# XJTU-Power-AI/charginghub-env

Measured on AMD Instinct MI355X. Metric: env-steps/sec at 65 536 parallel envs, higher is better.
Workload: dtype f64; 1 GPU; 65536 envs x hub [20 fast, 25 slow] (BASELINE.json configs[3]), fcev_permeate 0.01, random policy resident in HBM, reset every 96 steps, Philox streams; envs_per_gpu=65536, obs_dim=13, act_dim=47, work_order=XCD-aware (tiles, tail and level workgroups in contiguous eighths per XCD), graph=on, collective=none

## Files before the change

### charginghub-env_amd/csrc/chub_kernels.hip

```cpp
#include <hip/hip_runtime.h>
#include <hip/hip_ext.h>
#include <stdint.h>

#include "chub_device.h"
#include "chub_plan.h"

namespace chub {

typedef uint32_t u32x4 __attribute__((ext_vector_type(4)));
typedef uint32_t u32x2 __attribute__((ext_vector_type(2)));

__device__ __forceinline__ bool in_group(const StepArgs &sa, int64_t env) { return !sa.env_mask || sa.env_mask[env] != 0; }
__device__ __forceinline__ uint32_t env_clk(const StepArgs &sa, int64_t n_envs, int64_t env) {
    return sa.env_clk[(int64_t) (sa.tick & 1u) * n_envs + env];
}
__device__ __forceinline__ int64_t range_len(const StepArgs &sa) { return (int64_t) sa.env_hi - sa.env_lo + 1; }
__device__ __forceinline__ bool range_unit(const StepArgs &sa, int64_t i, int segments, int &seg, int64_t &env) {
    const int64_t R = range_len(sa);
    if (i >= (int64_t) segments * R) return false;
    seg = (i >= R ? 1 : 0) + (i >= 2 * R ? 1 : 0);
    env = sa.env_lo + (i - (int64_t) seg * R);
    return true;
}

// ... 2617 lines not shown

struct NoMid {
    __device__ __forceinline__ void operator()() {}
    __device__ __forceinline__ void at1() {}
    __device__ __forceinline__ void at2() {}
    __device__ __forceinline__ void at3() {}
};
__device__ __forceinline__ uint32_t hv_count_rate(float rate, uint32_t n) {
    const int c = (int) roundf(rate * (float) n);
    return (uint32_t) (c < 0 ? 0 : (c > 255 ? 255 : c));
}
__device__ __forceinline__ uint32_t hv_count_env(const EnvParamArrays &ep, uint32_t e, int t, uint32_t lev) {
    return hv_count_rate(ep.hv_rate[e], (uint32_t) ep.hv_idx[(uint32_t) t * (uint32_t) kLevels + lev]);
}

template <bool RESET, int MODE, bool MULTI, bool FUSED = false, typename Mid = NoMid, int EB = kEnvBlock, bool TAPE = false, bool EP = false, int PAIR = 0>
__device__ __forceinline__ void env_tail(const DevCtx *__restrict__ ctx, const StepArgs &sa, const int env, const bool live,
                                         const double *s_pv, const double *s_wd, const double *s_pv_now, const double *s_wd_now,
                                         const double *s_hy, const uint8_t *s_hv, float *s_out, const int env_block, const TailArgs &ta,
                                         const u32x4 *s_rec, const int local_env, const int env0_fused, const int rows_fused,
                                         const TailIn &pre, const bool use_pre, Mid &mid, TailNext *nx = nullptr, const TailArgs *ta2 = nullptr) {
    static_assert(PAIR == 0 || (!RESET && MODE == MODE_PHILOX && !MULTI && !FUSED && !TAPE && !EP), "pairs: the lock-step PHILOX step of the stand-alone tail");
    const HubParams &hp = ctx->hp;
    const EnvArrays &ev = ctx->ev;
    const CompatRng &cr = ctx->cr;
    const Tables &tb = ctx->tb;
    const int64_t N = hp.n_envs;
    constexpr bool multi = MULTI;
    const uint32_t my_clk = (multi && env < (int) N) ? env_clk(sa, N, env) : 0u;
    if (multi && env < (int) N)
        sa.env_clk[(int64_t) ((sa.tick + 1u) & 1u) * N + env] = (uint16_t) (!live ? my_clk : (RESET ? 0u : clk_next(my_clk)));
    const int t_now = multi ? clk_t(my_clk) : sa.t;
    const int t_next = RESET ? 0 : (t_now + 1) % 96;
    const bool draw_price = multi ? ((my_clk >> 8) & 3u) == 0u : sa.draw_price != 0;
    const double price_last = multi ? tb.price[RESET ? 95 : t_now] : sa.price_last;
    const double price_prev = multi ? tb.price[(t_now + 95) % 96] : sa.price_prev;
#define TAB_PV(d) (multi ? tb.pvT[t_next * 100 + (d)] : s_pv[d])
// ... 9 lines not shown
    CHUB_STAMP(0);
#if CHUB_TRACE
    {
        uint32_t n_ = n32;
        asm volatile("" : "+s"(n_));
        CHUB_STAMP(1);
    }
#endif
    double st_pv = 0.0, st_wd = 0.0, st_hy = 0.0, st_pv_now = 0.0, st_wd_now = 0.0;
    uint32_t st_hv = 0;
    const double sin_t = multi ? tb.sin96[t_next] : ta.sin_t;
    const int32_t tel_word = hp.telemetry;
    const bool tel_on = (tel_word & 1) != 0;
    const bool ep_on = (tel_word & 2) != 0;
    if (!FUSED) {
        const int i = threadIdx.x;
        if (PAIR == 2) {
            st_pv = nx->st_pv;
            st_wd = nx->st_wd;
        } else if (!multi) {
            if (i < 100) st_pv = ta.pv_row[i];
            if (i < 150) st_wd = ta.wd_row[i];
            if (!RESET) {
                if (i < 100) st_pv_now = ta.pv_row_now[i];
                if (i < 150) st_wd_now = ta.wd_row_now[i];
            }
            if (PAIR == 1) {
                nx->st_pv = nx->st_wd = 0.0;
                if (i < 100) nx->st_pv = ta2->pv_row[i];
                if (i < 150) nx->st_wd = ta2->wd_row[i];
            }
        }
        if (!RESET && PAIR != 2) {
            if (!EP && i < 102) st_hy = ta.hy_table[i];
            if (MODE == MODE_COMPAT && !EP && !multi && !sa.hv_tape && i < kLevels / 4) st_hv = ((CHUB_G(const uint32_t)) tb.cnt_hv)[sa.t * (kLevels / 4) + i];
        }
    }
    constexpr bool tick_late = MODE == MODE_PHILOX && !RESET && !TAPE;
    const bool tick_now = MODE == MODE_PHILOX && (!tick_late || sa.fresh != 0);
    PhiloxCtx px{ta.key[0], ta.key[1], tick_now ? sa.tick + sload_u32(ta.tick_base, 0) : sa.tick, ta.gid0 + (uint32_t) env};
    double cap = 0.0, in_price_noise = 0.0;
    double ou_pv = 0.0, ou_wd = 0.0, ou_price = 0.0, z_pv = 0.0, z_wd = 0.0, z_pr = 0.0;
    float a_el_f = 0.0f, a_fc_f = 0.0f, P0f = 0.0f, P1f = 0.0f, mn0 = 0.0f, mx0 = 0.0f, mn1 = 0.0f, mx1 = 0.0f;
    int pv_day = 0, wd_day = 0, q_len = 0, hv_line = 0, F0i = 0, F1i = 0, ln0 = 0, ln1 = 0, hv_lev = 0, hv_arrive = 0;
    u32x4 drw_raw = {0u, 0u, 0u, 0u};
    uint32_t drw_n = 0u, hvw0 = 0u, hvw1 = 0u;
    const bool have_pre = (FUSED || PAIR == 2) && use_pre;
    double p_v_h_max = 0.0, p_cells = 0.0, p_rc_cells = 0.0, p_cap_mass = 0.0, p_rc_cap_mass = 0.0, p_init_soc = 0.0, p_hydro_loss = 0.0;
    double p_fc_max_power = 0.0, p_renew_fluct1 = 0.0, p_price_fluct1 = 0.0;
// ... 4 lines not shown
            p_renew_fluct1 = pr[PRM_RENEW_FLUCT1 * n32 + e32];
            p_price_fluct1 = pr[PRM_PRICE_FLUCT1 * n32 + e32];
            if (RESET) {
                p_init_soc = pr[PRM_INIT_SOC * n32 + e32];
            } else {
                p_v_h_max = pr[PRM_V_H_MAX * n32 + e32];
                p_cells = pr[PRM_CELLS * n32 + e32];
                p_rc_cells = pr[PRM_RC_CELLS * n32 + e32];
                p_rc_cap_mass = pr[PRM_RC_CAP_MASS * n32 + e32];
                p_hydro_loss = pr[PRM_HYDRO_LOSS * n32 + e32];
                p_fc_max_power = pr[PRM_FC_MAX_POWER * n32 + e32];
            }
        }
        if (have_pre) {
            ou_pv = pre.ou_pv; ou_wd = pre.ou_wd; ou_price = pre.ou_price; in_price_noise = pre.price_noise;
        } else {
            ou_pv = ta.ou[e32];
            ou_wd = ta.ou[n32 + e32];
            ou_price = ta.ou[2u * n32 + e32];
            in_price_noise = ta.price_noise[e32];
        }
        if (PAIR == 2) {
            const u32x4 v0 = nx->r0, v1 = nx->r1;
            mn0 = __uint_as_float(v0.x); P0f = __uint_as_float(v0.y); mx0 = __uint_as_float(v0.z); ln0 = pkd_line(v0.w); F0i = pkd_flow(v0.w);
            mn1 = __uint_as_float(v1.x); P1f = __uint_as_float(v1.y); mx1 = __uint_as_float(v1.z); ln1 = pkd_line(v1.w); F1i = pkd_flow(v1.w);
        } else if (!FUSED) {
            const StationRec r0 = rec_load(ta.rec, e32), r1 = rec_load(ta.rec, n32 + e32);
            mn0 = r0.mn; P0f = r0.chg; mx0 = r0.mx; ln0 = pkd_line(r0.pkd); F0i = pkd_flow(r0.pkd);
            mn1 = r1.mn; P1f = r1.chg; mx1 = r1.mx; ln1 = pkd_line(r1.pkd); F1i = pkd_flow(r1.pkd);
        }
        if (!RESET && have_pre) {
            a_el_f = pre.a_el; a_fc_f = pre.a_fc; cap = pre.cap;
            pv_day = pre.pv_day; wd_day = pre.wd_day; q_len = pre.q_len; hv_line = pre.hv_line;
        } else if (!RESET) {
            if (ta.tail_act) {
                typedef float f32x2_ __attribute__((ext_vector_type(2)));
                const f32x2_ tv = ((CHUB_G(const f32x2_)) ta.tail_act)[e32];
                a_el_f = tv.x;
                a_fc_f = tv.y;
            } else {
                const uint32_t ai = e32 * ta.act_dim + ta.s_tot;
                a_el_f = ta.actions[ai];
                a_fc_f = ta.actions[ai + 1u];
            }
            cap = ta.cap[e32];
            pv_day = ta.pv_day[e32];
            wd_day = ta.wd_day[e32];
            q_len = ta.q_len[e32];
            hv_line = ta.hv_line[e32];
        }
        if (MODE == MODE_COMPAT && !RESET && sa.hv_tape) {
            hvw0 = sa.hv_tape[e32 * (uint32_t) sa.hv_w];
            if (sa.hv_w > 1) hvw1 = sa.hv_tape[e32 * (uint32_t) sa.hv_w + 1u];
        }
        if (TAPE) {
            z_pv = sa.exo_z[e32 * 3u + 0u];
            z_wd = sa.exo_z[e32 * 3u + 1u];
            z_pr = sa.exo_z[e32 * 3u + 2u];
            if (!RESET) hv_arrive = (int) sa.hv_tape[e32 * (uint32_t) sa.hv_w];
        } else if (MODE == MODE_PHILOX && !RESET && !sa.fresh) {
            if (have_pre) {
                drw_raw = pre.drw;
                drw_n = pre.drw_n;
            } else {
                drw_raw = ((CHUB_G(const u32x4)) ta.drw)[e32];
                drw_n = ta.drw_cnt[e32];
            }
        } else if (MODE == MODE_PHILOX) {
            const U4 ow = px.block(SITE_OU, 0, 0);
            z_pv = (double) normal_from_word(tb.normal_icdf, tb.normal_tail, ow.v[0]);
            z_wd = (double) normal_from_word(tb.normal_icdf, tb.normal_tail, ow.v[1]);
            z_pr = (double) normal_from_word(tb.normal_icdf, tb.normal_tail, ow.v[2]);
            if (!RESET) {
                hv_lev = (int) (px.block(SITE_HV, 0, 0).v[0] % 1000u);
                hv_arrive = EP ? (int) hv_count_env(ctx->ep, e32, t_now, (uint32_t) hv_lev)
                               : (int) tb.cnt_hv[(uint32_t) t_now * (uint32_t) kLevels + (uint32_t) hv_lev];
            }
        } else {
            z_pv = sa.exo_z[e32 * 3u + 0u];
            z_wd = sa.exo_z[e32 * 3u + 1u];
            z_pr = sa.exo_z[e32 * 3u + 2u];
        }
        if (PAIR == 1) {
            typedef float f32x2_ __attribute__((ext_vector_type(2)));
            nx->r0 = ((CHUB_G(const u32x4)) ta2->rec)[e32];
            nx->r1 = ((CHUB_G(const u32x4)) ta2->rec)[n32 + e32];
            const f32x2_ tv = ((CHUB_G(const f32x2_)) ta2->tail_act)[e32];
            nx->in.a_el = tv.x;
            nx->in.a_fc = tv.y;
            nx->in.drw = ((CHUB_G(const u32x4)) ta2->drw)[e32];
            nx->in.drw_n = ta2->drw_cnt[e32];
        }
    }


    if (tick_late && !tick_now) {
        const uint32_t *tbp = ta.tick_base;
        asm volatile("" : "+s"(tbp) : : "memory");
        px.tick += sload_u32(tbp, 0);
    }
    if (!FUSED) {
        static_assert(EB >= 150, "one table element per lane");
        CHUB_STAMP(2);
        const int i = threadIdx.x;
        if (i < 100) ((double *) s_pv)[i] = st_pv;
        if (i < 150) ((double *) s_wd)[i] = st_wd;
        if (!RESET && PAIR != 2) {
            if (i < 100) ((double *) s_pv_now)[i] = st_pv_now;
            if (i < 150) ((double *) s_wd_now)[i] = st_wd_now;
            if (!EP && i < 102) ((double *) s_hy)[i] = st_hy;
            if (MODE == MODE_COMPAT && !EP && i < kLevels / 4) ((uint32_t *) s_hv)[i] = st_hv;
        }
        __syncthreads();
    }
    CHUB_STAMP(3);
    if (!TAPE && MODE == MODE_PHILOX && !RESET && !sa.fresh) {
        z_pv = (double) __uint_as_float(drw_raw.x);
        z_wd = (double) __uint_as_float(drw_raw.y);
        z_pr = (double) __uint_as_float(drw_raw.z);
        hv_arrive = (int) drw_n;
    }
    const int row_w = sa.obs_stride;
    auto flush_rows = [&]() {
        if (FUSED) {
            __builtin_amdgcn_fence(__ATOMIC_RELEASE, "wavefront");
            __builtin_amdgcn_wave_barrier();
// ... 6 lines not shown
                for (int i = (int) (threadIdx.x & 63u); i < quads; i += 64) ((f32x4 *) dst)[i] = ((const f32x4 *) s_out)[i];
                for (int i = (quads << 2) + (int) (threadIdx.x & 63u); i < total; i += 64) dst[i] = s_out[i];
            } else {
                for (int i = (int) (threadIdx.x & 63u); i < total; i += 64) dst[i] = s_out[i];
            }
            __builtin_amdgcn_fence(__ATOMIC_RELEASE, "wavefront");
            __builtin_amdgcn_wave_barrier();
            return;
        }
        __syncthreads();
        const int env0 = env_block * EB;
        const int rows = (int) N - env0 < EB ? (int) N - env0 : EB;
        float *dst = sa.obs + (size_t) env0 * (size_t) row_w;
        const int total = rows * row_w;
        if (MULTI && sa.env_mask && !__syncthreads_and((live || env >= (int) N) ? 1 : 0)) {
            for (int i = threadIdx.x; i < total; i += EB)
                if (in_group(sa, env0 + i / row_w)) dst[i] = s_out[i];
        } else if ((((uintptr_t) dst) & 15u) == 0) {
            typedef float f32x4 __attribute__((ext_vector_type(4)));
            const int quads = total >> 2;
            for (int i = threadIdx.x; i < quads; i += EB) ((f32x4 *) dst)[i] = ((const f32x4 *) s_out)[i];
            for (int i = (quads << 2) + threadIdx.x; i < total; i += EB) dst[i] = s_out[i];
        } else {
            for (int i = threadIdx.x; i < total; i += EB) dst[i] = s_out[i];
        }
    };
    const double *hy_env = (MODE == MODE_COMPAT || EP) ? (const double *) ev.hy_env + (size_t) e32 * 102u : nullptr;
    (void) hy_env;
    double hy_req_pre = 0.0;
    if ((MODE == MODE_COMPAT || EP) && !RESET && live) {
        int rq = (int) ceil((((double) a_el_f + 1) / 2) * 100);
        rq = rq < 0 ? 0 : (rq > 101 ? 101 : rq);
        hy_req_pre = hy_env[rq];
    }
    const double cap_mass = HP_E(cap_mass, p_cap_mass);
    double store_soc = 0.0, reward = 0.0, in_re_pv = 0.0, in_re_wd = 0.0, in_price_next = 0.0, total_mass_need = 0.0;
    double re_pv = 0.0, re_wd = 0.0, price_next = 0.0;
    int arrive = 0;
    uint32_t fold_n = 0;
    do {
    if (!live) break;

    const bool hv_walked = MODE == MODE_COMPAT && sa.hv_tape != nullptr;
    CompatStream rs;
    if (MODE == MODE_COMPAT && !RESET && !hv_walked) rs.load(cr, sa.rng_cur, env);

    if (RESET) {
        if (MODE == MODE_COMPAT || TAPE) {
            pv_day = sa.exo_days[e32 * 2u + 0u];
            wd_day = sa.exo_days[e32 * 2u + 1u];
        } else {
            const U4 o = px.block(SITE_DAY, 0, 0);
            pv_day = (int) (o.v[0] % 100u);
            wd_day = (int) (o.v[1] % 150u);
        }
        ev.pv_day[e32] = (int16_t) pv_day;
// ... 131 lines not shown
        if (draw_price) {
            price_next = ou_sample(ou_price, .1, 0.005, z_pr) * HP_E(price_fluct1, p_price_fluct1);
            ev.ou[2u * n32 + e32] = ou_price;
            ev.price_noise[e32] = price_next;
            if (PAIR == 1) nx->in.price_noise = price_next;
            price_next += price_last;
        } else {
            price_next = price_last + in_price_noise;
            if (PAIR == 1) nx->in.price_noise = in_price_noise;
        }
    }
    if (MODE == MODE_COMPAT && !RESET && !hv_walked) rs.store(cr, sa.rng_cur, env);
    } while (0);

    CHUB_STAMP(4);
    mid();
    if (FUSED && live) {
        const u32x4 v0 = s_rec[2 * local_env], v1 = s_rec[2 * local_env + 1];
        mn0 = __uint_as_float(v0.x); P0f = __uint_as_float(v0.y); mx0 = __uint_as_float(v0.z); ln0 = pkd_line(v0.w); F0i = pkd_flow(v0.w);
        mn1 = __uint_as_float(v1.x); P1f = __uint_as_float(v1.y); mx1 = __uint_as_float(v1.z); ln1 = pkd_line(v1.w); F1i = pkd_flow(v1.w);
    }

    do {
    if (!live) break;
    if (!RESET) {
        const double a_el = ((double) a_el_f + 1) / 2;
        const double a_fc = ((double) a_fc_f + 1) / 2;
        const double P0 = (double) P0f, P1 = (double) P1f;
        const double F0 = (double) F0i, F1 = (double) F1i;
        double re_new_power = in_re_wd + in_re_pv;
        const double charging_power = 0.0 + P0 + P1;
// ... 85 lines not shown
        const double hy_loss = -6 / 1000.0 * hy_to_use;
        const double real_price_dollar = in_price_next / 4;
        const double income_evs_fast = 0.42 / 4 * P0 - real_price_dollar * e0;
        const double income_evs_slow = 0.21 / 4 * P1 - real_price_dollar * e1;
        const double income_evs = income_evs_fast + income_evs_slow;
        const double income_evs_serve = 0.8 * (0.0 + F0 + F1);
        const double income_hys = 6 / 1000.0 * hy_use;
        const double not_meet_loss = -10 / 1000.0 * not_meet;
        const double hy_cost = -real_price_dollar * hydrogen_power;
        reward = DIV_K(income_hys + income_evs + income_evs_serve + hy_cost + 1 * hy_loss + not_meet_loss, 50);
        if (tel_on) {
            CHUB_TEL(0, act_el); CHUB_TEL(1, flow); CHUB_TEL(2, all_power_second); CHUB_TEL(4, cap);
            CHUB_TEL(5, total_mass_need); CHUB_TEL(6, hy_use); CHUB_TEL(7, not_meet); CHUB_TEL(8, fc_power);
            CHUB_TEL(9, hy_to_use); CHUB_TEL(10, used_renew); CHUB_TEL(13, hydrogen_power);
            CHUB_TEL(14, income_hys + income_evs + income_evs_serve + hy_cost); CHUB_TEL(15, reward);
            CHUB_TEL(19, (double) arrive); CHUB_TEL(20, (double) hv_line); CHUB_TEL(21, (double) q_len + (double) fold_n);
            CHUB_TEL(24, e0); CHUB_TEL(25, e1); CHUB_TEL(26, ev_power_sum);
            CHUB_TEL(27, in_price_next);
        }
        if (ep_on) {
            CHUB_G(double) lv = ctx->es.live;
            const size_t nn = n32, ee = e32;
            const double init_soc = EP ? ctx->ep.prm[PRM_INIT_SOC * n32 + e32] : hp.init_soc;
            double col[kEpCount];
            col[EPC_RETURN] = lv[EPC_RETURN * nn + ee] + reward;
            col[EPC_INCOME] = lv[EPC_INCOME * nn + ee] + (income_hys + income_evs + income_evs_serve + hy_cost);
            col[EPC_DRAW_ELE] = lv[EPC_DRAW_ELE * nn + ee] + ((e0 + e1) + hydrogen_power);
            col[EPC_LENGTH] = lv[EPC_LENGTH * nn + ee] + 1.0;
            col[EPC_DEVIATION] = fabs(store_soc - init_soc);
            col[EPC_TEST_PENALTY] = fabs(col[EPC_DEVIATION] * cap_mass / 1000 / 0.2);
            col[EPC_END_SOC] = store_soc;
// ... 8 lines not shown
            }
        }
        }
    }

    ev.cap[e32] = cap;
    if (PAIR == 1) {
        nx->in.ou_pv = ou_pv;
        nx->in.ou_wd = ou_wd;
        nx->in.ou_price = ou_price;
        nx->in.cap = cap;
        nx->in.pv_day = pv_day;
        nx->in.wd_day = wd_day;
    }

    float *obs = s_out + (FUSED ? (int) (threadIdx.x & 63u) : (int) threadIdx.x) * row_w;
    double *o64 = tel_on ? (double *) ev.obs64 + (size_t) e32 * hp.obs_dim : nullptr;
    int n = 0;
#define CHUB_OBS(v)                    \
    do {                               \
        const double v_ = (v);         \
        obs[n] = (float) v_;           \
        if (o64) o64[n] = v_;          \
        n++;                           \
    } while (0)
    CHUB_OBS(sin_t);
    CHUB_OBS(div_c(price_next - hp.price_mean, hp.price_std, hp.rc_price_std));
    if (hp.S[0] > 0) {
        const double half_range = (double) hp.transformer_limit[0] / 2, rc_hr = hp.rc_half_range[0];
        CHUB_OBS(div_c((double) mn0 - half_range, half_range, rc_hr));
        CHUB_OBS(div_c((double) P0f - half_range, half_range, rc_hr));
// ... 16 lines not shown
        if (sa.done_f32) {
            obs[n] = (float) reward;
            obs[n + 1] = dn ? 1.0f : 0.0f;
        } else {
            sa.reward[(size_t) e32 * sa.reward_stride] = (float) reward;
            if (sa.done) sa.done[e32] = (uint8_t) (dn ? 1 : 0);
            if (sa.done_f32) sa.done_f32[(size_t) e32 * sa.reward_stride] = dn ? 1.0f : 0.0f;
        }
    } else if (MULTI && sa.done_f32) {
        obs[n] = sa.reward[(size_t) e32 * sa.reward_stride];
        obs[n + 1] = sa.done_f32[(size_t) e32 * sa.reward_stride];
    }
    if (tel_on) {
        ev.reward64[e32] = reward;
        CHUB_TEL(3, store_soc); CHUB_TEL(16, re_pv); CHUB_TEL(17, re_wd); CHUB_TEL(18, price_next);
        CHUB_TEL(22, (double) pv_day); CHUB_TEL(23, (double) wd_day);
        CHUB_TEL(28, (double) mn0); CHUB_TEL(29, (double) P0f); CHUB_TEL(30, (double) mx0); CHUB_TEL(31, (double) ln0); CHUB_TEL(32, (double) F0i);
        CHUB_TEL(33, (double) mn1); CHUB_TEL(34, (double) P1f); CHUB_TEL(35, (double) mx1); CHUB_TEL(36, (double) ln1); CHUB_TEL(37, (double) F1i);
    }
    } while (0);
    CHUB_STAMP(5);
    mid.at3();
    if (MULTI) {
        if (RESET && sa.final_obs && live) {
            const float *row = sa.obs + (size_t) e32 * (size_t) row_w;
            float *fin = sa.final_obs + (size_t) e32 * (size_t) hp.obs_dim;
            for (int j = 0; j < hp.obs_dim; j++) fin[j] = row[j];
        }
        if (sa.tick_note && live) sa.tick_note[e32] = CHUB_TICK(hp, sa.tick);
        if (!RESET && sa.done_mask) {
            const bool dn = live && (t_now + 1) >= 96;
            if (env < (int) N) sa.done_mask[e32] = (uint8_t) (dn ? 1 : 0);
            const unsigned long long fired = __ballot(dn);
            if ((threadIdx.x & 63u) == 0u && fired != 0ull) atomicAdd(sa.done_count, (uint32_t) __popcll(fired));
        }
    }
    flush_rows();
#if CHUB_TRACE
    CHUB_STAMP(6);
    asm volatile("s_waitcnt vmcnt(0)" ::: "memory");
    CHUB_STAMP(7);
    CHUB_STAMP_REAL(9);
    if (!FUSED && sa.stamps_env && threadIdx.x == 0) for (int i = 0; i < 10; i++) sa.stamps_env[(size_t) env_block * 16 + i] = stamp_[i];
#endif
#undef TAB_PV
#undef TAB_WD
#undef TAB_PV_NOW
#undef TAB_WD_NOW
#undef TAB_HY
#undef TAB_HV
#undef HP_E
}

template <bool RESET, bool MULTI, bool EP = false>
__device__ __forceinline__ void level_block(const DevCtx *__restrict__ ctx, const StepArgs &sa, const int64_t u, const int line_known = -1) {
    const HubParams &hp = ctx->hp;
    const int64_t N = hp.n_envs;
    if (u >= 3 * N) return;
// ... 78 lines not shown
    const HubParams &hp = ctx->hp;
    const Tables &tb = ctx->tb;
    PhiloxCtx px{hp.key[0], hp.key[1], tick, (uint32_t) (hp.env_id0 + e)};
    const U4 ow = px.block(SITE_OU, 0, 0);
    const uint32_t hv_lev = px.block(SITE_HV, 0, 0).v[0] % 1000u;
    u32x4 d;
    d.x = __float_as_uint(normal_from_word(tb.normal_icdf, tb.normal_tail, ow.v[0]));
    d.y = __float_as_uint(normal_from_word(tb.normal_icdf, tb.normal_tail, ow.v[1]));
    d.z = __float_as_uint(normal_from_word(tb.normal_icdf, tb.normal_tail, ow.v[2]));
    const uint32_t cnt = (uint32_t) tb.cnt_hv[(uint32_t) t * (uint32_t) kLevels + hv_lev];
    d.w = cnt != 0u ? __float_as_uint(soc_from_word(tb.soc_d_icdf, px.block(SITE_HVSOC, 0, 0).v[0])) : 0u;
    ((CHUB_G(u32x4)) drw)[e] = d;
    cnt_out[e] = (uint8_t) cnt;
}

__device__ __forceinline__ bool level_lane(const uint32_t jb, const uint32_t n32, const int nb_env, const uint32_t xcd, int64_t &u) {
    const uint32_t per = n32 >> 3;
    if (xcd && (n32 & 2047u) == 0u && ((uint32_t) nb_env & 7u) == 0u) {
        const uint32_t x = jb & 7u, i = jb >> 3, wpx = per / kEnvBlock;
        const uint32_t seg = i / wpx;
        u = (int64_t) seg * n32 + (int64_t) (x * per + (i - seg * wpx) * kEnvBlock + threadIdx.x);
        return seg < 3u;
    }
    u = (int64_t) jb * kEnvBlock + threadIdx.x;
    return u < 3 * (int64_t) n32;
}

__global__ __launch_bounds__(kEnvBlock) void k_pair_draws(const DevCtx *__restrict__ ctx, StepArgs sa, PairArgs pr, uint32_t xcd) {
    const HubParams &hp = ctx->hp;
    const uint32_t n32 = (uint32_t) hp.n_envs;
    int64_t u;
    if (!level_lane(blockIdx.x, n32, 8, xcd, u)) return;
    const uint32_t tick1 = CHUB_TICK(hp, sa.tick + 1u);
    if (u < 2 * (int64_t) n32) {
        const int kk = u >= (int64_t) n32 ? 1 : 0;
        const int want = dk_want(ctx->st.pk[sa.tick & 1u][u]);
        pr.pkraw[u] = draw_raw_levels(hp, ctx->tb, tick1, sa.t + 1, kk, u - (int64_t) kk * n32, want, hp.type[kk] == 0);
    } else {
        const uint32_t e = (uint32_t) (u - 2 * (int64_t) n32);
        draw_env_pre(ctx, tick1 - 1u, sa.t, e, pr.drw_out[0], pr.cnt_out[0]);
        draw_env_pre(ctx, tick1, sa.t + 1, e, pr.drw_out[1], pr.cnt_out[1]);
    }
}

template <bool MORE>
__global__ __launch_bounds__(kEnvBlock) void k_env_pair(const DevCtx *__restrict__ ctx, StepArgs sa, StepArgs sb, TailArgs ta, TailArgs tb2, PairArgs pr,
                                                        int nb_env) {
    __shared__ double s_pv[100], s_wd[150], s_pv_now[100], s_wd_now[150], s_hy[102], s_pv2[100], s_wd2[150];
    __shared__ __attribute__((aligned(16))) float s_out[2][kEnvBlock * 16];
    if ((int) blockIdx.x >= nb_env) {
        const HubParams &hp = ctx->hp;
        const uint32_t n32 = (uint32_t) hp.n_envs;
        int64_t u;
        if (!level_lane(blockIdx.x - (uint32_t) nb_env, n32, nb_env, ta.xcd, u)) return;
        if (!MORE) {
            level_block<false, false>(ctx, sb, u);
            if (u < 2 * (int64_t) n32) {
                const int kk = u >= (int64_t) n32 ? 1 : 0;
                ctx->st.pk[sb.tick & 1u][u] = dk_make(pr.pkraw[u], pkd_line(pr.rec_a[4u * (uint32_t) u + 3u]), hp.type[kk] == 0);
            } else {
                const uint32_t e = (uint32_t) (u - 2 * (int64_t) n32);
                ((CHUB_G(u32x4)) ctx->ev.drw[sb.tick & 1u])[e] = ((CHUB_G(const u32x4)) pr.drw_in[1])[e];
                ctx->ev.drw_cnt[sb.tick & 1u][e] = pr.cnt_in[1][e];
            }
            return;
        }
        const uint32_t tick2 = CHUB_TICK(hp, sb.tick + 1u);
        if (u < 2 * (int64_t) n32) {
            const int kk = u >= (int64_t) n32 ? 1 : 0;
            const bool fast = hp.type[kk] == 0;
            const int64_t env_ = u - (int64_t) kk * n32;
            const int line_now = pkd_line(ctx->st.rec[4u * (uint32_t) u + 3u]);
            const uint32_t dk = draw_decoded_levels(hp, ctx->tb, tick2, sb.t + 1, kk, env_, line_now, fast);
            ctx->st.pk[(sb.tick + 1u) & 1u][u] = dk;
            pr.pkraw[u] = draw_raw_levels(hp, ctx->tb, tick2 + 1u, sb.t + 2, kk, env_, dk_want(dk), fast);
        } else {
            const uint32_t e = (uint32_t) (u - 2 * (int64_t) n32);
            draw_env_pre(ctx, tick2, sb.t + 1, e, pr.drw_out[0], pr.cnt_out[0]);
            draw_env_pre(ctx, tick2 + 1u, sb.t + 2, e, pr.drw_out[1], pr.cnt_out[1]);
        }
        return;
    }
    const int blk = (int) xcd_order(blockIdx.x, (uint32_t) nb_env, ta.xcd);
    const int env = blk * kEnvBlock + (int) threadIdx.x;
    const bool live = env < (int) ta.n_envs;
    TailIn none;
    TailNext nx;
    NoMid nomid;
    env_tail<false, MODE_PHILOX, false, false, NoMid, kEnvBlock, false, false, 1>(ctx, sa, env, live, s_pv, s_wd, s_pv_now, s_wd_now, s_hy, nullptr, s_out[0], blk, ta,
                                                                                  nullptr, 0, 0, 0, none, false, nomid, &nx, &tb2);
    env_tail<false, MODE_PHILOX, false, false, NoMid, kEnvBlock, false, false, 2>(ctx, sb, env, live, s_pv2, s_wd2, s_pv, s_wd, s_hy, nullptr, s_out[1], blk, tb2,
                                                                                  nullptr, 0, 0, 0, nx.in, true, nomid, &nx, nullptr);
}

__global__ __launch_bounds__(256) void k_env_walk(const DevCtx *__restrict__ ctx, StepArgs sa, TailArgs ta, StepArgs sw, int nb_env) {
    __shared__ __attribute__((aligned(16))) uint32_t lds[32 * 256 + 4 * kWalkStageWords];
    if ((int) blockIdx.x >= nb_env) {
        __builtin_amdgcn_s_setprio(3);
        compat_walk_block<false>(ctx, sw, blockIdx.x - (uint32_t) nb_env, lds, lds + 32 * 256);
        return;
    }
    double *s_pv = (double *) lds, *s_wd = s_pv + 100, *s_pv_now = s_wd + 150, *s_wd_now = s_pv_now + 100, *s_hy = s_wd_now + 150;
    uint8_t *s_hv = (uint8_t *) (s_hy + 102 + 2);
    float *s_out = (float *) (s_hv + 1008);
    static_assert((602 + 2) * 8 + 1008 + kEnvBlock * 16 * 4 <= 32 * 256 * 4 && kLevels <= 1008, "the tail's LDS inside the walk's");
    const int env = (int) blockIdx.x * kEnvBlock + (int) threadIdx.x;
    TailIn none;
// ... 1580 lines not shown
template void launch_env<false>(EnvForm, const HubParams &, const DevCtx *, const StepArgs &, hipStream_t, hipEvent_t, hipEvent_t, const PackedPtrs &);

void launch_env_walk(const HubParams &hp, const DevCtx *ctx, const StepArgs &sa, const StepArgs &sw, hipStream_t stream, hipEvent_t ev0, hipEvent_t ev1,
                     const PackedPtrs &pp) {
    const TailArgs ta = make_tail_args(*pp.ev, *pp.st, hp, sa, pp, false);
    const int nb_env = (int) ((hp.n_envs + kEnvBlock - 1) / kEnvBlock);
    const unsigned nb = (unsigned) nb_env + (unsigned) ((hp.n_envs + 255) / 256);
    CHUB_LAUNCH(k_env_walk, dim3(nb), dim3(kEnvBlock), stream, ev0, ev1, ctx, sa, ta, sw, nb_env);
}

void launch_pair(const HubParams &hp, const DevCtx *ctx, const StepArgs &sa_in, const StepArgs &sb_in, hipStream_t stream, const PackedPtrs &pp,
                 const PairBufs &pb, int sel, bool chain_start, bool more) {
    StepArgs sa = sa_in, sb = sb_in;
    const int64_t N = hp.n_envs;
    const int nb_env = (int) ((N + kEnvBlock - 1) / kEnvBlock);
    const unsigned nb_lev = (unsigned) ((3 * N + kEnvBlock - 1) / kEnvBlock);
    PairArgs pr;
    pr.rec_a = (CHUB_G(const uint32_t)) pb.rec_a;
    pr.pkraw = (CHUB_G(uint64_t)) pb.pkraw;
    for (int q = 0; q < 2; q++) {
        pr.drw_in[q] = (CHUB_G(const uint32_t)) pb.drw[sel][q];
        pr.cnt_in[q] = (CHUB_G(const uint8_t)) pb.cnt[sel][q];
        pr.drw_out[q] = (CHUB_G(uint32_t)) pb.drw[sel ^ 1][q];
        pr.cnt_out[q] = (CHUB_G(uint8_t)) pb.cnt[sel ^ 1][q];
    }
    const uint32_t xcd = hp.xcd ? 1u : 0u;
    if (chain_start) {
        launch_levels(sa.fresh ? LEVELS_DRAW : LEVELS_NONE, ctx, sa, stream);
        PairArgs p0 = pr;
        for (int q = 0; q < 2; q++) {
            p0.drw_out[q] = (CHUB_G(uint32_t)) pb.drw[sel][q];
            p0.cnt_out[q] = (CHUB_G(uint8_t)) pb.cnt[sel][q];
        }
        hipLaunchKernelGGL(k_pair_draws, dim3(nb_lev), dim3(kEnvBlock), 0, stream, ctx, sa, p0, xcd);
    }
    sa.fresh = 0;
    sb.fresh = 0;
    const uint32_t nb = (uint32_t) ((N + hp.epb - 1) / hp.epb);
    PackedArgs pa = make_packed_args(hp, sa, pp);
    pa.rec = (CHUB_G(uint32_t)) pb.rec_a;
    pa.tail_act = (CHUB_G(float)) pb.tail_act_a;
    hipLaunchKernelGGL((k_slot_packed<kPackedBlock, kSlotsPerLane, false, false, false, false>), dim3(nb), dim3(kPackedBlock), 0, stream, ctx, sa, pa);
    PackedArgs pa2 = make_packed_args(hp, sb, pp);
    pa2.pk = (CHUB_G(const uint32_t)) (const void *) pb.pkraw;
    pa2.rec_prev = (CHUB_G(const uint32_t)) pb.rec_a;
    hipLaunchKernelGGL((k_slot_packed<kPackedBlock, kSlotsPerLane, false, false, false, false, false, true>), dim3(nb), dim3(kPackedBlock), 0, stream, ctx,
                       sb, pa2);
    TailArgs ta = make_tail_args(*pp.ev, *pp.st, hp, sa, pp, false), tb2 = make_tail_args(*pp.ev, *pp.st, hp, sb, pp, false);
    ta.rec = (CHUB_G(uint32_t)) pb.rec_a;
    ta.tail_act = (CHUB_G(const float)) pb.tail_act_a;
    ta.drw = pr.drw_in[0];
    ta.drw_cnt = pr.cnt_in[0];
    tb2.drw = pr.drw_in[1];
    tb2.drw_cnt = pr.cnt_in[1];
    if (more) hipLaunchKernelGGL(k_env_pair<true>, dim3((unsigned) nb_env + nb_lev), dim3(kEnvBlock), 0, stream, ctx, sa, sb, ta, tb2, pr, nb_env);
    else hipLaunchKernelGGL(k_env_pair<false>, dim3((unsigned) nb_env + nb_lev), dim3(kEnvBlock), 0, stream, ctx, sa, sb, ta, tb2, pr, nb_env);
}

__global__ void k_tick_advance(uint32_t *tick_base, uint32_t by) { *tick_base += by; }


__global__ void k_expand_bits(int64_t n_envs, int S, int W, const uint64_t *__restrict__ bits, const float *__restrict__ tail,
                              float *__restrict__ actions) {
    const uint32_t A = (uint32_t) S + 2u;
    const uint32_t total = (uint32_t) n_envs * A;
    for (uint32_t i = blockIdx.x * blockDim.x + threadIdx.x; i < total; i += gridDim.x * blockDim.x) {
        const uint32_t env = i / A;
        const uint32_t j = i - env * A;
        float v;
        if (j < (uint32_t) S) v = ((bits[(size_t) env * (size_t) W + (j >> 6)] >> (j & 63u)) & 1ull) ? 1.0f : -1.0f;
        else v = tail[env * 2u + (j - (uint32_t) S)];
// ... 251 lines not shown
```

### charginghub-env_amd/csrc/chub_runtime.cpp

```cpp
#include <hip/hip_runtime.h>
#include <math.h>
#include <stdint.h>
#include <stdio.h>
#include <string.h>
#include <stdlib.h>

#include <algorithm>
#include <map>
#include <string>
#include <vector>

#include "../../include/chub.h"
#include "chub_device.h"
#include "chub_plan.h"
#include "chub_policy.h"
#include "chub_critic.h"
#include "chub_adam.h"

namespace chub {
template <bool RESET>
void launch_slot(const CallPlan &cp, const HubParams &hp, const LaunchPlan &lp, const DevCtx *ctx, const StepArgs &sa, hipStream_t stream,
                 const PackedPtrs &pp, hipEvent_t ev0, hipEvent_t ev1);
void launch_check_ttab(const DevCtx *ctx, uint32_t *d_mismatch, hipStream_t stream);
void launch_build_cls_soc(const DevCtx *ctx, float *d_out, hipStream_t stream);
// ... 1652 lines not shown
        const StepCall c2 = step_call(nullptr, batches[(i + 1) % n_batches], nullptr, packed_out(e, packed2[(i + 1) & 1]), 0);
        StepArgs sa, sb;
        if (const int rc = fill_args(e, c1, 2, all, e->tick + 1u, s, sa)) return rc;
        {
            const int t0 = e->t, pc0 = e->price_count;
            const bool pd0 = e->predrawn;
            e->t = t0 + 1;
            e->price_count = pc0 + 1;
            e->predrawn = true;
            const int rc = fill_args(e, c2, 2, all, e->tick + 2u, s, sb);
            e->t = t0;
            e->price_count = pc0;
            e->predrawn = pd0;
            if (rc) return rc;
        }
        launch_pair(e->hp, e->d_ctx, sa, sb, s, packed_ptrs(e), e->pair, sel, p == 0, p + 1 < n_pairs);
        if (hipGetLastError() != hipSuccess) {
            e->predrawn = false;
            return fail(CHUB_ERR_HIP, "a pair of steps could not be launched");
        }
        e->tick += 2u;
        advance_clocks(e, c1, 2, 2);
        sel ^= 1;
    }
    return note_served(e, nullptr, 2, s);
}

int chub_run_steps(chub_env *e, chub_comm *comm, const float *const *d_action_batches, int n_batches, float *const *d_packed2,
                   float *const *d_gathered2, float *d_reset_obs, int64_t first_step, int64_t n_steps, void *stream) {
    if (!e || !d_action_batches || n_batches <= 0 || !d_packed2 || !d_packed2[0] || !d_packed2[1] || !d_reset_obs || first_step < 0 ||
// ... 3623 lines not shown
```

Measured before the change: 2.747 billion env-steps/s.

## Split pair tail across two role halves of a doubled workgroup

The paired-step kernel now launches workgroups twice as wide. One half (role 1) runs the first part of each env's tail: loading tables, computing renewables, price and mass need, and writing them to shared memory. The other half (role 2) loads station records, actions and hydrogen tables, then takes over the rest of the step after a barrier. This splits each env's serial work across two wavefront groups and lets more memory loads be in flight at once. It adds barriers and shared-memory hand-over traffic. The level and draw kernels also use the larger block size.

```diff
diff --git a/charginghub-env_amd/csrc/chub_kernels.hip b/charginghub-env_amd/csrc/chub_kernels.hip
--- a/charginghub-env_amd/csrc/chub_kernels.hip
+++ b/charginghub-env_amd/csrc/chub_kernels.hip
@@ -2655,13 +2655,22 @@
     return hv_count_rate(ep.hv_rate[e], (uint32_t) ep.hv_idx[(uint32_t) t * (uint32_t) kLevels + lev]);
 }
 
-template <bool RESET, int MODE, bool MULTI, bool FUSED = false, typename Mid = NoMid, int EB = kEnvBlock, bool TAPE = false, bool EP = false, int PAIR = 0>
+struct PairSplit {
+    double *s_pv2, *s_wd2;
+    double *hand;
+};
+template <bool RESET, int MODE, bool MULTI, bool FUSED = false, typename Mid = NoMid, int EB = kEnvBlock, bool TAPE = false, bool EP = false, int PAIR = 0,
+          int ROLE = 0>
 __device__ __forceinline__ void env_tail(const DevCtx *__restrict__ ctx, const StepArgs &sa, const int env, const bool live,
                                          const double *s_pv, const double *s_wd, const double *s_pv_now, const double *s_wd_now,
                                          const double *s_hy, const uint8_t *s_hv, float *s_out, const int env_block, const TailArgs &ta,
                                          const u32x4 *s_rec, const int local_env, const int env0_fused, const int rows_fused,
-                                         const TailIn &pre, const bool use_pre, Mid &mid, TailNext *nx = nullptr, const TailArgs *ta2 = nullptr) {
+                                         const TailIn &pre, const bool use_pre, Mid &mid, TailNext *nx = nullptr, const TailArgs *ta2 = nullptr,
+                                         const PairSplit *ps = nullptr) {
     static_assert(PAIR == 0 || (!RESET && MODE == MODE_PHILOX && !MULTI && !FUSED && !TAPE && !EP), "pairs: the lock-step PHILOX step of the stand-alone tail");
+    static_assert(ROLE == 0 || PAIR != 0, "roles: the halves of a pair's steps");
+    const int tid = ROLE ? (int) (threadIdx.x & (uint32_t) (EB - 1)) : (int) threadIdx.x;
+    (void) tid;
     const HubParams &hp = ctx->hp;
     const EnvArrays &ev = ctx->ev;
     const CompatRng &cr = ctx->cr;
@@ -2701,11 +2710,11 @@
     const bool tel_on = (tel_word & 1) != 0;
     const bool ep_on = (tel_word & 2) != 0;
     if (!FUSED) {
-        const int i = threadIdx.x;
+        const int i = tid;
         if (PAIR == 2) {
             st_pv = nx->st_pv;
             st_wd = nx->st_wd;
-        } else if (!multi) {
+        } else if (!multi && ROLE != 2) {
             if (i < 100) st_pv = ta.pv_row[i];
             if (i < 150) st_wd = ta.wd_row[i];
             if (!RESET) {
@@ -2719,7 +2728,7 @@
             }
         }
         if (!RESET && PAIR != 2) {
-            if (!EP && i < 102) st_hy = ta.hy_table[i];
+            if (ROLE != 1 && !EP && i < 102) st_hy = ta.hy_table[i];
             if (MODE == MODE_COMPAT && !EP && !multi && !sa.hv_tape && i < kLevels / 4) st_hv = ((CHUB_G(const uint32_t)) tb.cnt_hv)[sa.t * (kLevels / 4) + i];
         }
     }
@@ -2754,7 +2763,7 @@
         }
         if (have_pre) {
             ou_pv = pre.ou_pv; ou_wd = pre.ou_wd; ou_price = pre.ou_price; in_price_noise = pre.price_noise;
-        } else {
+        } else if (ROLE != 2) {
             ou_pv = ta.ou[e32];
             ou_wd = ta.ou[n32 + e32];
             ou_price = ta.ou[2u * n32 + e32];
@@ -2764,7 +2773,7 @@
             const u32x4 v0 = nx->r0, v1 = nx->r1;
             mn0 = __uint_as_float(v0.x); P0f = __uint_as_float(v0.y); mx0 = __uint_as_float(v0.z); ln0 = pkd_line(v0.w); F0i = pkd_flow(v0.w);
             mn1 = __uint_as_float(v1.x); P1f = __uint_as_float(v1.y); mx1 = __uint_as_float(v1.z); ln1 = pkd_line(v1.w); F1i = pkd_flow(v1.w);
-        } else if (!FUSED) {
+        } else if (!FUSED && ROLE != 1) {
             const StationRec r0 = rec_load(ta.rec, e32), r1 = rec_load(ta.rec, n32 + e32);
             mn0 = r0.mn; P0f = r0.chg; mx0 = r0.mx; ln0 = pkd_line(r0.pkd); F0i = pkd_flow(r0.pkd);
             mn1 = r1.mn; P1f = r1.chg; mx1 = r1.mx; ln1 = pkd_line(r1.pkd); F1i = pkd_flow(r1.pkd);
@@ -2773,7 +2782,8 @@
             a_el_f = pre.a_el; a_fc_f = pre.a_fc; cap = pre.cap;
             pv_day = pre.pv_day; wd_day = pre.wd_day; q_len = pre.q_len; hv_line = pre.hv_line;
         } else if (!RESET) {
-            if (ta.tail_act) {
+            if (ROLE == 1) {
+            } else if (ta.tail_act) {
                 typedef float f32x2_ __attribute__((ext_vector_type(2)));
                 const f32x2_ tv = ((CHUB_G(const f32x2_)) ta.tail_act)[e32];
                 a_el_f = tv.x;
@@ -2783,11 +2793,13 @@
                 a_el_f = ta.actions[ai];
                 a_fc_f = ta.actions[ai + 1u];
             }
-            cap = ta.cap[e32];
-            pv_day = ta.pv_day[e32];
-            wd_day = ta.wd_day[e32];
-            q_len = ta.q_len[e32];
-            hv_line = ta.hv_line[e32];
+            if (ROLE != 1) cap = ta.cap[e32];
+            if (ROLE != 2) {
+                pv_day = ta.pv_day[e32];
+                wd_day = ta.wd_day[e32];
+                q_len = ta.q_len[e32];
+                hv_line = ta.hv_line[e32];
+            }
         }
         if (MODE == MODE_COMPAT && !RESET && sa.hv_tape) {
             hvw0 = sa.hv_tape[e32 * (uint32_t) sa.hv_w];
@@ -2802,7 +2814,7 @@
             if (have_pre) {
                 drw_raw = pre.drw;
                 drw_n = pre.drw_n;
-            } else {
+            } else if (ROLE != 2) {
                 drw_raw = ((CHUB_G(const u32x4)) ta.drw)[e32];
                 drw_n = ta.drw_cnt[e32];
             }
@@ -2823,33 +2835,45 @@
         }
         if (PAIR == 1) {
             typedef float f32x2_ __attribute__((ext_vector_type(2)));
-            nx->r0 = ((CHUB_G(const u32x4)) ta2->rec)[e32];
-            nx->r1 = ((CHUB_G(const u32x4)) ta2->rec)[n32 + e32];
-            const f32x2_ tv = ((CHUB_G(const f32x2_)) ta2->tail_act)[e32];
-            nx->in.a_el = tv.x;
-            nx->in.a_fc = tv.y;
-            nx->in.drw = ((CHUB_G(const u32x4)) ta2->drw)[e32];
-            nx->in.drw_n = ta2->drw_cnt[e32];
-        }
-    }
-
-
-    if (tick_late && !tick_now) {
+            if (ROLE != 1) {
+                nx->r0 = ((CHUB_G(const u32x4)) ta2->rec)[e32];
+                nx->r1 = ((CHUB_G(const u32x4)) ta2->rec)[n32 + e32];
+                const f32x2_ tv = ((CHUB_G(const f32x2_)) ta2->tail_act)[e32];
+                nx->in.a_el = tv.x;
+                nx->in.a_fc = tv.y;
+            }
+            if (ROLE != 2) {
+                nx->in.drw = ((CHUB_G(const u32x4)) ta2->drw)[e32];
+                nx->in.drw_n = ta2->drw_cnt[e32];
+            }
+        }
+    }
+
+
+    if (tick_late && !tick_now && ROLE != 2) {
         const uint32_t *tbp = ta.tick_base;
         asm volatile("" : "+s"(tbp) : : "memory");
         px.tick += sload_u32(tbp, 0);
     }
-    if (!FUSED) {
+    if (!FUSED && !(ROLE != 0 && PAIR == 2)) {
         static_assert(EB >= 150, "one table element per lane");
         CHUB_STAMP(2);
-        const int i = threadIdx.x;
-        if (i < 100) ((double *) s_pv)[i] = st_pv;
-        if (i < 150) ((double *) s_wd)[i] = st_wd;
+        const int i = tid;
+        if (ROLE != 2) {
+            if (i < 100) ((double *) s_pv)[i] = st_pv;
+            if (i < 150) ((double *) s_wd)[i] = st_wd;
+        }
         if (!RESET && PAIR != 2) {
-            if (i < 100) ((double *) s_pv_now)[i] = st_pv_now;
-            if (i < 150) ((double *) s_wd_now)[i] = st_wd_now;
-            if (!EP && i < 102) ((double *) s_hy)[i] = st_hy;
+            if (ROLE != 2) {
+                if (i < 100) ((double *) s_pv_now)[i] = st_pv_now;
+                if (i < 150) ((double *) s_wd_now)[i] = st_wd_now;
+            }
+            if (ROLE != 1 && !EP && i < 102) ((double *) s_hy)[i] = st_hy;
             if (MODE == MODE_COMPAT && !EP && i < kLevels / 4) ((uint32_t *) s_hv)[i] = st_hv;
+        }
+        if (ROLE == 1) {
+            if (i < 100) ps->s_pv2[i] = nx->st_pv;
+            if (i < 150) ps->s_wd2[i] = nx->st_wd;
         }
         __syncthreads();
     }
@@ -2886,15 +2910,15 @@
         float *dst = sa.obs + (size_t) env0 * (size_t) row_w;
         const int total = rows * row_w;
         if (MULTI && sa.env_mask && !__syncthreads_and((live || env >= (int) N) ? 1 : 0)) {
-            for (int i = threadIdx.x; i < total; i += EB)
+            for (int i = tid; i < total; i += EB)
                 if (in_group(sa, env0 + i / row_w)) dst[i] = s_out[i];
         } else if ((((uintptr_t) dst) & 15u) == 0) {
             typedef float f32x4 __attribute__((ext_vector_type(4)));
             const int quads = total >> 2;
-            for (int i = threadIdx.x; i < quads; i += EB) ((f32x4 *) dst)[i] = ((const f32x4 *) s_out)[i];
-            for (int i = (quads << 2) + threadIdx.x; i < total; i += EB) dst[i] = s_out[i];
+            for (int i = tid; i < quads; i += EB) ((f32x4 *) dst)[i] = ((const f32x4 *) s_out)[i];
+            for (int i = (quads << 2) + tid; i < total; i += EB) dst[i] = s_out[i];
         } else {
-            for (int i = threadIdx.x; i < total; i += EB) dst[i] = s_out[i];
+            for (int i = tid; i < total; i += EB) dst[i] = s_out[i];
         }
     };
     const double *hy_env = (MODE == MODE_COMPAT || EP) ? (const double *) ev.hy_env + (size_t) e32 * 102u : nullptr;
@@ -2911,7 +2935,7 @@
     int arrive = 0;
     uint32_t fold_n = 0;
     do {
-    if (!live) break;
+    if (!live || ROLE == 2) break;
 
     const bool hv_walked = MODE == MODE_COMPAT && sa.hv_tape != nullptr;
     CompatStream rs;
@@ -3073,7 +3097,46 @@
     } while (0);
 
     CHUB_STAMP(4);
+    if (ROLE == 1) {
+        double *h = ps->hand;
+        h[tid] = in_re_pv;
+        h[EB + tid] = in_re_wd;
+        h[2 * EB + tid] = in_price_next;
+        h[3 * EB + tid] = total_mass_need;
+        h[4 * EB + tid] = re_pv;
+        h[5 * EB + tid] = re_wd;
+        h[6 * EB + tid] = price_next;
+    }
     mid();
+    CHUB_STAMP(10);
+    if (ROLE == 1) {
+        if (PAIR == 1) {
+            nx->in.ou_pv = ou_pv;
+            nx->in.ou_wd = ou_wd;
+            nx->in.ou_price = ou_price;
+            nx->in.pv_day = pv_day;
+            nx->in.wd_day = wd_day;
+        }
+        if (tel_on && live) {
+            CHUB_TEL(19, (double) arrive); CHUB_TEL(20, (double) hv_line); CHUB_TEL(21, (double) q_len + (double) fold_n);
+            CHUB_TEL(22, (double) pv_day); CHUB_TEL(23, (double) wd_day);
+        }
+#if CHUB_TRACE
+        CHUB_STAMP_REAL(9);
+        if (sa.stamps_env && tid == 0) for (int i = 0; i < 11; i++) sa.stamps_env[((size_t) env_block * 4 + (PAIR - 1)) * 16 + i] = stamp_[i];
+#endif
+        return;
+    }
+    if (ROLE == 2 && live) {
+        const double *h = ps->hand;
+        in_re_pv = h[tid];
+        in_re_wd = h[EB + tid];
+        in_price_next = h[2 * EB + tid];
+        total_mass_need = h[3 * EB + tid];
+        re_pv = h[4 * EB + tid];
+        re_wd = h[5 * EB + tid];
+        price_next = h[6 * EB + tid];
+    }
     if (FUSED && live) {
         const u32x4 v0 = s_rec[2 * local_env], v1 = s_rec[2 * local_env + 1];
         mn0 = __uint_as_float(v0.x); P0f = __uint_as_float(v0.y); mx0 = __uint_as_float(v0.z); ln0 = pkd_line(v0.w); F0i = pkd_flow(v0.w);
@@ -3189,7 +3252,9 @@
             CHUB_TEL(5, total_mass_need); CHUB_TEL(6, hy_use); CHUB_TEL(7, not_meet); CHUB_TEL(8, fc_power);
             CHUB_TEL(9, hy_to_use); CHUB_TEL(10, used_renew); CHUB_TEL(13, hydrogen_power);
             CHUB_TEL(14, income_hys + income_evs + income_evs_serve + hy_cost); CHUB_TEL(15, reward);
-            CHUB_TEL(19, (double) arrive); CHUB_TEL(20, (double) hv_line); CHUB_TEL(21, (double) q_len + (double) fold_n);
+            if (ROLE != 2) {
+                CHUB_TEL(19, (double) arrive); CHUB_TEL(20, (double) hv_line); CHUB_TEL(21, (double) q_len + (double) fold_n);
+            }
             CHUB_TEL(24, e0); CHUB_TEL(25, e1); CHUB_TEL(26, ev_power_sum);
             CHUB_TEL(27, in_price_next);
         }
@@ -3228,7 +3293,7 @@
         nx->in.wd_day = wd_day;
     }
 
-    float *obs = s_out + (FUSED ? (int) (threadIdx.x & 63u) : (int) threadIdx.x) * row_w;
+    float *obs = s_out + (FUSED ? (int) (threadIdx.x & 63u) : tid) * row_w;
     double *o64 = tel_on ? (double *) ev.obs64 + (size_t) e32 * hp.obs_dim : nullptr;
     int n = 0;
 #define CHUB_OBS(v)                    \
@@ -3275,7 +3340,9 @@
     if (tel_on) {
         ev.reward64[e32] = reward;
         CHUB_TEL(3, store_soc); CHUB_TEL(16, re_pv); CHUB_TEL(17, re_wd); CHUB_TEL(18, price_next);
-        CHUB_TEL(22, (double) pv_day); CHUB_TEL(23, (double) wd_day);
+        if (ROLE != 2) {
+            CHUB_TEL(22, (double) pv_day); CHUB_TEL(23, (double) wd_day);
+        }
         CHUB_TEL(28, (double) mn0); CHUB_TEL(29, (double) P0f); CHUB_TEL(30, (double) mx0); CHUB_TEL(31, (double) ln0); CHUB_TEL(32, (double) F0i);
         CHUB_TEL(33, (double) mn1); CHUB_TEL(34, (double) P1f); CHUB_TEL(35, (double) mx1); CHUB_TEL(36, (double) ln1); CHUB_TEL(37, (double) F1i);
     }
@@ -3296,13 +3363,14 @@
             if ((threadIdx.x & 63u) == 0u && fired != 0ull) atomicAdd(sa.done_count, (uint32_t) __popcll(fired));
         }
     }
-    flush_rows();
+    if (!(ROLE == 2 && PAIR == 1)) flush_rows();
 #if CHUB_TRACE
     CHUB_STAMP(6);
     asm volatile("s_waitcnt vmcnt(0)" ::: "memory");
     CHUB_STAMP(7);
     CHUB_STAMP_REAL(9);
-    if (!FUSED && sa.stamps_env && threadIdx.x == 0) for (int i = 0; i < 10; i++) sa.stamps_env[(size_t) env_block * 16 + i] = stamp_[i];
+    const size_t stamp_row = PAIR ? (size_t) env_block * 4 + (PAIR - 1) + (ROLE == 2 ? 2 : 0) : (size_t) env_block;
+    if (!FUSED && sa.stamps_env && tid == 0) for (int i = 0; i < 11; i++) sa.stamps_env[stamp_row * 16 + i] = stamp_[i];
 #endif
 #undef TAB_PV
 #undef TAB_WD
@@ -3411,23 +3479,29 @@
     cnt_out[e] = (uint8_t) cnt;
 }
 
+template <int LB>
 __device__ __forceinline__ bool level_lane(const uint32_t jb, const uint32_t n32, const int nb_env, const uint32_t xcd, int64_t &u) {
     const uint32_t per = n32 >> 3;
-    if (xcd && (n32 & 2047u) == 0u && ((uint32_t) nb_env & 7u) == 0u) {
-        const uint32_t x = jb & 7u, i = jb >> 3, wpx = per / kEnvBlock;
+    if (xcd && (n32 & (8u * LB - 1u)) == 0u && ((uint32_t) nb_env & 7u) == 0u) {
+        const uint32_t x = jb & 7u, i = jb >> 3, wpx = per / LB;
         const uint32_t seg = i / wpx;
-        u = (int64_t) seg * n32 + (int64_t) (x * per + (i - seg * wpx) * kEnvBlock + threadIdx.x);
+        u = (int64_t) seg * n32 + (int64_t) (x * per + (i - seg * wpx) * LB + threadIdx.x);
         return seg < 3u;
     }
-    u = (int64_t) jb * kEnvBlock + threadIdx.x;
+    u = (int64_t) jb * LB + threadIdx.x;
     return u < 3 * (int64_t) n32;
 }
 
-__global__ __launch_bounds__(kEnvBlock) void k_pair_draws(const DevCtx *__restrict__ ctx, StepArgs sa, PairArgs pr, uint32_t xcd) {
+#ifndef CHUB_PAIR_SPLIT
+#define CHUB_PAIR_SPLIT 1
+#endif
+constexpr int kPairBlock = CHUB_PAIR_SPLIT ? 2 * kEnvBlock : kEnvBlock;
+
+__global__ __launch_bounds__(kPairBlock) void k_pair_draws(const DevCtx *__restrict__ ctx, StepArgs sa, PairArgs pr, uint32_t xcd) {
     const HubParams &hp = ctx->hp;
     const uint32_t n32 = (uint32_t) hp.n_envs;
     int64_t u;
-    if (!level_lane(blockIdx.x, n32, 8, xcd, u)) return;
+    if (!level_lane<kPairBlock>(blockIdx.x, n32, 8, xcd, u)) return;
     const uint32_t tick1 = CHUB_TICK(hp, sa.tick + 1u);
     if (u < 2 * (int64_t) n32) {
         const int kk = u >= (int64_t) n32 ? 1 : 0;
@@ -3441,15 +3515,10 @@
 }
 
 template <bool MORE>
-__global__ __launch_bounds__(kEnvBlock) void k_env_pair(const DevCtx *__restrict__ ctx, StepArgs sa, StepArgs sb, TailArgs ta, TailArgs tb2, PairArgs pr,
-                                                        int nb_env) {
-    __shared__ double s_pv[100], s_wd[150], s_pv_now[100], s_wd_now[150], s_hy[102], s_pv2[100], s_wd2[150];
-    __shared__ __attribute__((aligned(16))) float s_out[2][kEnvBlock * 16];
-    if ((int) blockIdx.x >= nb_env) {
+__device__ __forceinline__ void pair_levels(const DevCtx *__restrict__ ctx, const StepArgs &sb, const PairArgs &pr, const int64_t u) {
+    {
         const HubParams &hp = ctx->hp;
         const uint32_t n32 = (uint32_t) hp.n_envs;
-        int64_t u;
-        if (!level_lane(blockIdx.x - (uint32_t) nb_env, n32, nb_env, ta.xcd, u)) return;
         if (!MORE) {
             level_block<false, false>(ctx, sb, u);
             if (u < 2 * (int64_t) n32) {
@@ -3476,18 +3545,95 @@
             draw_env_pre(ctx, tick2, sb.t + 1, e, pr.drw_out[0], pr.cnt_out[0]);
             draw_env_pre(ctx, tick2 + 1u, sb.t + 2, e, pr.drw_out[1], pr.cnt_out[1]);
         }
+    }
+}
+
+struct PairMid {
+    __device__ __forceinline__ void operator()() { __syncthreads(); }
+    __device__ __forceinline__ void at1() {}
+    __device__ __forceinline__ void at2() {}
+    __device__ __forceinline__ void at3() {}
+};
+
+template <bool MORE>
+__global__ __launch_bounds__(kPairBlock) void k_env_pair(const DevCtx *__restrict__ ctx, StepArgs sa, StepArgs sb, TailArgs ta, TailArgs tb2, PairArgs pr,
+                                                         int nb_env) {
+    __shared__ double s_pv[100], s_wd[150], s_pv_now[100], s_wd_now[150], s_hy[102], s_pv2[100], s_wd2[150];
+    __shared__ __attribute__((aligned(16))) float s_out[2][kEnvBlock * 16];
+    if ((int) blockIdx.x >= nb_env) {
+#if CHUB_TRACE
+        CHUB_STAMP_DECL(16);
+        CHUB_STAMP_REAL(8);
+#endif
+        int64_t u;
+        if (level_lane<kPairBlock>(blockIdx.x - (uint32_t) nb_env, (uint32_t) ctx->hp.n_envs, nb_env, ta.xcd, u)) pair_levels<MORE>(ctx, sb, pr, u);
+#if CHUB_TRACE
+        asm volatile("s_waitcnt vmcnt(0)" ::: "memory");
+        CHUB_STAMP_REAL(9);
+        if (sa.stamps_env && threadIdx.x == 0) {
+            const size_t row = (size_t) nb_env * 4 + (blockIdx.x - (uint32_t) nb_env);
+            sa.stamps_env[row * 16 + 8] = stamp_[8];
+            sa.stamps_env[row * 16 + 9] = stamp_[9];
+        }
+#endif
         return;
     }
     const int blk = (int) xcd_order(blockIdx.x, (uint32_t) nb_env, ta.xcd);
+    TailIn none;
+#if CHUB_PAIR_SPLIT
+    __shared__ double s_hand[7 * kEnvBlock];
+    static_assert(sizeof(s_out[1]) >= 7 * kEnvBlock * sizeof(double), "A1's hand-over inside the second step's rows");
+    const int role = __builtin_amdgcn_readfirstlane((int) (threadIdx.x / kEnvBlock));
+    const int lane = (int) (threadIdx.x & (uint32_t) (kEnvBlock - 1));
+    const int env = blk * kEnvBlock + lane;
+    const bool live = env < (int) ta.n_envs;
+    TailNext nx = TailNext();
+    PairMid pm;
+    const PairSplit p1{s_pv2, s_wd2, (double *) s_out[1]}, p2{nullptr, nullptr, s_hand};
+    if (role == 0) {
+        env_tail<false, MODE_PHILOX, false, false, PairMid, kEnvBlock, false, false, 1, 1>(ctx, sa, env, live, s_pv, s_wd, s_pv_now, s_wd_now, s_hy, nullptr, s_out[0],
+                                                                                          blk, ta, nullptr, 0, 0, 0, none, false, pm, &nx, &tb2, &p1);
+        env_tail<false, MODE_PHILOX, false, false, PairMid, kEnvBlock, false, false, 2, 1>(ctx, sb, env, live, s_pv2, s_wd2, s_pv, s_wd, s_hy, nullptr, s_out[1],
+                                                                                          blk, tb2, nullptr, 0, 0, 0, nx.in, true, pm, &nx, nullptr, &p2);
+#if CHUB_TRACE
+        CHUB_STAMP_DECL(16);
+        CHUB_STAMP(5);
+#endif
+        const int env0 = blk * kEnvBlock, row_w = sa.obs_stride;
+        const int rows = (int) ta.n_envs - env0 < kEnvBlock ? (int) ta.n_envs - env0 : kEnvBlock;
+        float *dst = sa.obs + (size_t) env0 * (size_t) row_w;
+        const float *src = s_out[0];
+        const int total = rows * row_w;
+        if ((((uintptr_t) dst) & 15u) == 0) {
+            typedef float f32x4 __attribute__((ext_vector_type(4)));
+            const int quads = total >> 2;
+            for (int i = lane; i < quads; i += kEnvBlock) ((f32x4 *) dst)[i] = ((const f32x4 *) src)[i];
+            for (int i = (quads << 2) + lane; i < total; i += kEnvBlock) dst[i] = src[i];
+        } else {
+            for (int i = lane; i < total; i += kEnvBlock) dst[i] = src[i];
+        }
+#if CHUB_TRACE
+        CHUB_STAMP(6);
+        asm volatile("s_waitcnt vmcnt(0)" ::: "memory");
+        CHUB_STAMP(7);
+        if (sa.stamps_env && lane == 0) for (int i = 5; i < 8; i++) sa.stamps_env[((size_t) blk * 4 + 1) * 16 + i] = stamp_[i];
+#endif
+        return;
+    }
+    env_tail<false, MODE_PHILOX, false, false, PairMid, kEnvBlock, false, false, 1, 2>(ctx, sa, env, live, s_pv, s_wd, s_pv_now, s_wd_now, s_hy, nullptr, s_out[0], blk,
+                                                                                      ta, nullptr, 0, 0, 0, none, false, pm, &nx, &tb2, &p1);
+    env_tail<false, MODE_PHILOX, false, false, PairMid, kEnvBlock, false, false, 2, 2>(ctx, sb, env, live, s_pv2, s_wd2, s_pv, s_wd, s_hy, nullptr, s_out[1], blk,
+                                                                                      tb2, nullptr, 0, 0, 0, nx.in, true, pm, &nx, nullptr, &p2);
+#else
     const int env = blk * kEnvBlock + (int) threadIdx.x;
     const bool live = env < (int) ta.n_envs;
-    TailIn none;
     TailNext nx;
     NoMid nomid;
     env_tail<false, MODE_PHILOX, false, false, NoMid, kEnvBlock, false, false, 1>(ctx, sa, env, live, s_pv, s_wd, s_pv_now, s_wd_now, s_hy, nullptr, s_out[0], blk, ta,
                                                                                   nullptr, 0, 0, 0, none, false, nomid, &nx, &tb2);
     env_tail<false, MODE_PHILOX, false, false, NoMid, kEnvBlock, false, false, 2>(ctx, sb, env, live, s_pv2, s_wd2, s_pv, s_wd, s_hy, nullptr, s_out[1], blk, tb2,
                                                                                   nullptr, 0, 0, 0, nx.in, true, nomid, &nx, nullptr);
+#endif
 }
 
 __global__ __launch_bounds__(256) void k_env_walk(const DevCtx *__restrict__ ctx, StepArgs sa, TailArgs ta, StepArgs sw, int nb_env) {
@@ -5098,7 +5244,7 @@
     StepArgs sa = sa_in, sb = sb_in;
     const int64_t N = hp.n_envs;
     const int nb_env = (int) ((N + kEnvBlock - 1) / kEnvBlock);
-    const unsigned nb_lev = (unsigned) ((3 * N + kEnvBlock - 1) / kEnvBlock);
+    const unsigned nb_lev = (unsigned) ((3 * N + kPairBlock - 1) / kPairBlock);
     PairArgs pr;
     pr.rec_a = (CHUB_G(const uint32_t)) pb.rec_a;
     pr.pkraw = (CHUB_G(uint64_t)) pb.pkraw;
@@ -5116,7 +5262,7 @@
             p0.drw_out[q] = (CHUB_G(uint32_t)) pb.drw[sel][q];
             p0.cnt_out[q] = (CHUB_G(uint8_t)) pb.cnt[sel][q];
         }
-        hipLaunchKernelGGL(k_pair_draws, dim3(nb_lev), dim3(kEnvBlock), 0, stream, ctx, sa, p0, xcd);
+        hipLaunchKernelGGL(k_pair_draws, dim3(nb_lev), dim3(kPairBlock), 0, stream, ctx, sa, p0, xcd);
     }
     sa.fresh = 0;
     sb.fresh = 0;
@@ -5137,8 +5283,8 @@
     ta.drw_cnt = pr.cnt_in[0];
     tb2.drw = pr.drw_in[1];
     tb2.drw_cnt = pr.cnt_in[1];
-    if (more) hipLaunchKernelGGL(k_env_pair<true>, dim3((unsigned) nb_env + nb_lev), dim3(kEnvBlock), 0, stream, ctx, sa, sb, ta, tb2, pr, nb_env);
-    else hipLaunchKernelGGL(k_env_pair<false>, dim3((unsigned) nb_env + nb_lev), dim3(kEnvBlock), 0, stream, ctx, sa, sb, ta, tb2, pr, nb_env);
+    if (more) hipLaunchKernelGGL(k_env_pair<true>, dim3((unsigned) nb_env + nb_lev), dim3(kPairBlock), 0, stream, ctx, sa, sb, ta, tb2, pr, nb_env);
+    else hipLaunchKernelGGL(k_env_pair<false>, dim3((unsigned) nb_env + nb_lev), dim3(kPairBlock), 0, stream, ctx, sa, sb, ta, tb2, pr, nb_env);
 }
 
 __global__ void k_tick_advance(uint32_t *tick_base, uint32_t by) { *tick_base += by; }
diff --git a/charginghub-env_amd/csrc/chub_runtime.cpp b/charginghub-env_amd/csrc/chub_runtime.cpp
--- a/charginghub-env_amd/csrc/chub_runtime.cpp
+++ b/charginghub-env_amd/csrc/chub_runtime.cpp
@@ -1690,6 +1690,9 @@
             e->predrawn = pd0;
             if (rc) return rc;
         }
+#if CHUB_TRACE
+        sa.stamps_env = sb.stamps_env = (unsigned long long *) g_stamps_env;
+#endif
         launch_pair(e->hp, e->d_ctx, sa, sb, s, packed_ptrs(e), e->pair, sel, p == 0, p + 1 < n_pairs);
         if (hipGetLastError() != hipSuccess) {
             e->predrawn = false;
```

Result: no change. 2.775 billion env-steps/s, median of 6 (+1.0%).
